# facebookresearch/dmc-net

Measured on AMD Instinct MI355X. Metric: clips/sec (3-seg 224x224) DMC-gen+ResNet-18 train step, higher is better.
Workload: dtype f32

## Files before the change

dmc-net_amd/csrc/conv_x3q.hip:

```cpp
#include "dmc_common.h"
#include "x3s_common.h"
#include <type_traits>
#include <utility>

using namespace dmc;
using namespace dmc::x3;

namespace {

constexpr int QBM = 256, QBN = 64;
constexpr int QWSLOT = 3 * QBN * 32;
constexpr int QWB = 3 * QWSLOT;
constexpr int QEP = 272, QETILE = 32 * QEP;

template <int NW_, int NPB_, int NT_>
struct QG {
    static constexpr int NW = NW_, NPB = NPB_, NT = NT_;
    static constexpr int NA = NW / 2;
    static constexpr int KP = (NT + NA - 1) / NA;
    static constexpr int PT = 3 * KP;
    static constexpr int KW = (18 + NA - 1) / NA;
    static constexpr int ZROW = 32 * NT;
    static constexpr int PSL = (ZROW + 1) * 32;
    static constexpr int PB = 3 * PSL;
// ... 404 lines not shown
int q_choose_tn(long M, int R) {
    const int forced = option(OPT_CONV_CFG);
    if (forced == 201) return 2;
    if (forced == 202) return 1;
    const long n2 = ((M + 255) / 256) * (R / QBN), n1 = ((M + 127) / 128) * (R / QBN);
    const double t2 = (double)((n2 + 255) / 256), t1 = 0.75 * (double)((n1 + 255) / 256);
    return t1 < t2 ? 1 : 2;
}

template <class P, int TN, class GEO>
int launch_q(const X3qArgs& a, hipStream_t s) {
    static LdsLimit lim;
    const hipError_t attr = lim.raise(reinterpret_cast<const void*>(&x3q_conv_kernel<P, TN, GEO>), GEO::LDS);
    if (attr != hipSuccess) return fail(DMC_E_LAUNCH, "x3q_conv: cannot raise the dynamic LDS limit: %s", hipGetErrorString(attr));
    constexpr int BM = 32 * GEO::NW / (2 / TN);
    dim3 grid((a.M + BM - 1) / BM, a.R / QBN);
    x3q_conv_kernel<P, TN, GEO><<<grid, GEO::NW * 64, GEO::LDS, s>>>(a);
    return check_launch("x3q_conv");
}

int q_patch_pixels_max128(long M, int W);
int q_variant(long M, int W, int R) {
    const int forced = option(OPT_CONV_CFG);
    const bool two_ok = q_patch_pixels_max128(M, W) <= QGTwo::ZROW;
    if (forced == 201) return 0;
    if (forced == 202) return 1;
    if (forced == 203 && two_ok) return 2;
    if (forced != 204 && two_ok && ((M + 127) / 128) * (R / QBN) >= 512) return 2;
    return q_choose_tn(M, R) == 2 ? 0 : 1;
}
int q_block_pixels(int variant) { return variant == 0 ? 256 : 128; }


struct X3qWgArgs {
    const void* xq;
    const void* dys;
    float* part;
    int N, OH, Cin, Cout;
    unsigned plane_bytes;
    int steps, per_group, tiles_ci;
};

template <int OW_, int R, int HP_>
struct QWgGeom {
    static constexpr int PW = OW_ + 1;
    static constexpr int D1 = 3, D0 = 2;
    static constexpr int XPL1 = ((D1 * R * PW + 3) / 8) * 8 + 4;
    static constexpr int XPL0 = ((D0 * R * PW + 3) / 8) * 8 + 4;
    static constexpr int NPX = R * OW_;
    static constexpr int NKB = (NPX + 15) / 16;
    static constexpr int DYT = ((NKB * 16 + 31) / 32) * 32;
    static constexpr int DYPL = ((DYT + 3) / 8) * 8 + 4;
    static constexpr int XI = (R * PW + 31) / 32;
    static constexpr int DI = DYT / 32;
    static constexpr int CLS_OFF[4] = {0, 4 * XPL0 * 32, 8 * XPL0 * 32, 8 * XPL0 * 32 + 4 * XPL1 * 32};
    static constexpr int SLB = 8 * XPL0 * 32 + 8 * XPL1 * 32;
    static constexpr int XBYTES = 3 * SLB, DYBYTES = 12 * DYPL * 32;
    static constexpr int LDS = XBYTES + 2 * DYBYTES;
    static_assert(HP_ % R == 0, "steps are whole groups of padded rows");
};

template <int OW_, int R, int HP_>
__global__ __launch_bounds__(768) void x3q_wgrad_kernel(X3qWgArgs a) {
    using G = QWgGeom<OW_, R, HP_>;
    constexpr int PW = G::PW, DYPL = G::DYPL, NKB = G::NKB;
    extern __shared__ __attribute__((aligned(1024))) char lds_qw[];
    const int tid = threadIdx.x, lane = tid & 63;
    const int wave = __builtin_amdgcn_readfirstlane(tid >> 6);
    const int l31 = lane & 31, khalf = lane >> 5, L = lane & 15, grp = (lane >> 4) & 1;
    const int quarter = wave & 3, trow = wave >> 2;
    const int wi = quarter & 1, wj = quarter >> 1;
    const int tci = blockIdx.x % a.tiles_ci, tco = blockIdx.x / a.tiles_ci;
    const unsigned lds0 = lds_addr_of(lds_qw);
    const int s_begin = blockIdx.y * a.per_group;
    const int s_end = s_begin + a.per_group < a.steps ? s_begin + a.per_group : a.steps;
    const u32x4 srd_x = make_srd(a.xq), srd_d = make_srd(a.dys);
    const int nch_in = a.Cin >> 4;
    const int tsl = wave >> 2, tch = wave & 3;
    const unsigned soff_d = (unsigned)(tsl * (a.Cout >> 4) + tco * 4 + tch) * a.plane_bytes;
    const unsigned dplane = lds0 + G::XBYTES + (unsigned)wave * DYPL * 32;
    const int lpx = lane >> 1;
    const unsigned lhalf = (unsigned)(lane & 1) << 4;

    auto pix_off = [&](int g, int x) -> unsigned {
        const int n = g / HP_, y = g - n * HP_ - 1;
        return (g >= 0 && n < a.N && y >= 0 && y < a.OH && x >= 0 && x < OW_) ? (unsigned)((n * a.OH + y) * OW_ + x) * 32u + lhalf : OOB;
    };
    auto issue_x = [&](int q) {
#pragma unroll
        for (int cls = 0; cls < 4; ++cls) {
            const int D = (cls >> 1) ? G::D1 : G::D0, xpl = (cls >> 1) ? G::XPL1 : G::XPL0;
            const int slot0 = (((q % D) + D) % D) * R;
            const unsigned soff_x = (unsigned)(tsl * 4 * nch_in + cls * nch_in + tci * 4 + tch) * a.plane_bytes;
            const unsigned xplane = lds0 + (unsigned)(tsl * G::SLB + G::CLS_OFF[cls] + tch * xpl * 32);
#pragma unroll
            for (int i = 0; i < G::XI; ++i) {
                const int px = 32 * i + lpx;
                const int r = px / PW, col = px - r * PW;
                if (px < R * PW) dma_buf16(srd_x, pix_off(R * q + r, col - 1), soff_x, xplane + (unsigned)(slot0 * PW + 32 * i) * 32u);
            }
        }
    };
    auto issue_dy = [&](int s, int buf) {
#pragma unroll
        for (int i = 0; i < G::DI; ++i) {
            const int p = 32 * i + lpx;
            const int r = p / OW_, x = p - r * OW_;
            dma_buf16(srd_d, p < G::NPX ? pix_off(R * s + r, x) : OOB, soff_d, dplane + (unsigned)buf * G::DYBYTES + (unsigned)(32 * i) * 32u);
        }
    };

    f32x16 acc[3];
#pragma unroll
    for (int t = 0; t < 3; ++t)
#pragma unroll
        for (int e = 0; e < 16; ++e) acc[t][e] = 0.f;

    if (s_begin < s_end) {
        issue_x(s_begin - 1);
        issue_x(s_begin);
        issue_dy(s_begin, 0);
    }
    asm volatile("s_waitcnt vmcnt(0)" ::: "memory");
    __builtin_amdgcn_s_barrier();
    const int py = trow != 1, da = trow == 0 ? -1 : 0;
    const int DR = (py ? G::D1 : G::D0) * R, xpl = py ? G::XPL1 : G::XPL0;
    const int cls_a = py ? G::CLS_OFF[3] : G::CLS_OFF[1];
    const int cls_b = py ? G::CLS_OFF[2] : G::CLS_OFF[0];
    lds_cptr const LB = (lds_cptr)lds_qw;
    int rr[NKB][2], xcol[NKB][2], dyoff[NKB][2];
#pragma unroll
    for (int kb = 0; kb < NKB; ++kb)
#pragma unroll
        for (int u = 0; u < 2; ++u) {
            int P = 16 * kb + 8 * khalf + 4 * u + (L >> 2);
            dyoff[kb][u] = (2 * wi + grp) * DYPL * 32 + G::XBYTES + (L & 3) * 8 + P * 32;
            if (P >= G::NPX) P = G::NPX - 1;
            rr[kb][u] = P / OW_;
            xcol[kb][u] = (2 * wj + grp) * xpl * 32 + (L & 3) * 8 + (P - rr[kb][u] * OW_) * 32;
        }
#pragma unroll 1
    for (int s = s_begin; s < s_end; ++s) {
        const int buf = (s - s_begin) & 1;
        issue_x(s + 1);
        if (s + 1 < s_end) issue_dy(s + 1, buf ^ 1);
        const int sb = (((R * s + da) % DR) + DR) % DR;
#pragma unroll
        for (int kb = 0; kb < NKB; ++kb) {
            int dyo[2], xa[2], xb[2];
#pragma unroll
            for (int u = 0; u < 2; ++u) {
                dyo[u] = dyoff[kb][u] + buf * G::DYBYTES;
                int slot = sb + rr[kb][u];
                slot = slot >= DR ? slot - DR : slot;
                const int xo = xcol[kb][u] + slot * PW * 32;
                xa[u] = xo + cls_a;
                xb[u] = xo + cls_b;
            }
            u32x4 A[3], B[3][3];
#pragma unroll
            for (int sl = 0; sl < 3; ++sl) {
                tr_read2(LB + dyo[0] + sl * 4 * DYPL * 32, LB + dyo[1] + sl * 4 * DYPL * 32, A[sl]);
                tr_read2(LB + xa[0] + sl * G::SLB, LB + xa[1] + sl * G::SLB, B[0][sl]);
                tr_read2(LB + xb[0] + sl * G::SLB + 32, LB + xb[1] + sl * G::SLB + 32, B[1][sl]);
                tr_read2(LB + xa[0] + sl * G::SLB + 32, LB + xa[1] + sl * G::SLB + 32, B[2][sl]);
            }
#pragma unroll
            for (int t = 0; t < 3; ++t) {
                acc[t] = mfma_bf16(A[0], B[t][2], acc[t]);
                acc[t] = mfma_bf16(A[2], B[t][0], acc[t]);
                acc[t] = mfma_bf16(A[1], B[t][1], acc[t]);
                acc[t] = mfma_bf16(A[0], B[t][1], acc[t]);
                acc[t] = mfma_bf16(A[1], B[t][0], acc[t]);
                acc[t] = mfma_bf16(A[0], B[t][0], acc[t]);
            }
        }
        asm volatile("s_waitcnt vmcnt(0) lgkmcnt(0)" ::: "memory");
        __builtin_amdgcn_s_barrier();
    }
    float* out = a.part + (size_t)blockIdx.y * a.Cout * 9 * a.Cin;
    const int ci = tci * 64 + 32 * wj + l31;
#pragma unroll
    for (int t = 0; t < 3; ++t)
#pragma unroll
        for (int e = 0; e < 16; ++e) {
            const int co = tco * 64 + 32 * wi + 8 * (e >> 2) + 4 * khalf + (e & 3);
            out[((size_t)co * 9 + 3 * trow + t) * a.Cin + ci] = acc[t][e];
        }
}

struct X3qWg1Args {
    const void* xq; const void* dys; float* part;
    int Cin, Cout; long Mq; unsigned plane_bytes; int steps, per_group, tiles_ci;
};
constexpr int W1PX = 64, W1PL = 68;
constexpr int W1TILE = 12 * W1PL * 32, W1LDS = 4 * W1TILE;

__global__ __launch_bounds__(256) void x3q_wgrad1_kernel(X3qWg1Args a) {
    extern __shared__ __attribute__((aligned(1024))) char lds_w1[];
    const int tid = threadIdx.x, lane = tid & 63;
    const int wave = __builtin_amdgcn_readfirstlane(tid >> 6);
    const int l31 = lane & 31, khalf = lane >> 5, L = lane & 15, grp = (lane >> 4) & 1;
    const int wi = wave & 1, wj = wave >> 1;
    const int tci = blockIdx.x % a.tiles_ci, tco = blockIdx.x / a.tiles_ci;
    const unsigned lds0 = lds_addr_of(lds_w1);
    const int s_begin = blockIdx.y * a.per_group;
    const int s_end = s_begin + a.per_group < a.steps ? s_begin + a.per_group : a.steps;
    const u32x4 srd_x = make_srd(a.xq), srd_d = make_srd(a.dys);
    const int nch_in = a.Cin >> 4, nch_out = a.Cout >> 4;
    const int lpx = lane >> 1;
    const unsigned lhalf = (unsigned)(lane & 1) << 4;
    auto issue = [&](int s, int buf) {
#pragma unroll
        for (int k = 0; k < 3; ++k) {
            const int pl = 3 * wave + k, sl = pl >> 2, ch = pl & 3;
#pragma unroll
            for (int i = 0; i < 2; ++i) {
                const long p = (long)s * W1PX + 32 * i + lpx;
                const unsigned voff = p < a.Mq ? (unsigned)p * 32u + lhalf : OOB;
                dma_buf16(srd_x, voff, (unsigned)(sl * 4 * nch_in + tci * 4 + ch) * a.plane_bytes,
                          lds0 + (unsigned)(buf * 2 * W1TILE + pl * W1PL * 32 + 32 * i * 32));
                dma_buf16(srd_d, voff, (unsigned)(sl * nch_out + tco * 4 + ch) * a.plane_bytes,
                          lds0 + (unsigned)(buf * 2 * W1TILE + W1TILE + pl * W1PL * 32 + 32 * i * 32));
            }
        }
    };
    f32x16 acc;
#pragma unroll
    for (int e = 0; e < 16; ++e) acc[e] = 0.f;
    if (s_begin < s_end) issue(s_begin, 0);
    asm volatile("s_waitcnt vmcnt(0)" ::: "memory");
    __builtin_amdgcn_s_barrier();
    lds_cptr const LB = (lds_cptr)lds_w1;
#pragma unroll 1
    for (int s = s_begin; s < s_end; ++s) {
        const int buf = (s - s_begin) & 1;
        if (s + 1 < s_end) issue(s + 1, buf ^ 1);
        const int xb = buf * 2 * W1TILE + (2 * wj + grp) * W1PL * 32 + (L & 3) * 8;
        const int db = buf * 2 * W1TILE + W1TILE + (2 * wi + grp) * W1PL * 32 + (L & 3) * 8;
#pragma unroll
        for (int kb = 0; kb < W1PX / 16; ++kb) {
            u32x4 A[3], B[3];
            const int P0 = 16 * kb + 8 * khalf + (L >> 2), P1 = P0 + 4;
#pragma unroll
            for (int sl = 0; sl < 3; ++sl) {
                tr_read2(LB + db + sl * 4 * W1PL * 32 + P0 * 32, LB + db + sl * 4 * W1PL * 32 + P1 * 32, A[sl]);
                tr_read2(LB + xb + sl * 4 * W1PL * 32 + P0 * 32, LB + xb + sl * 4 * W1PL * 32 + P1 * 32, B[sl]);
            }
            acc = mfma_bf16(A[0], B[2], acc);
            acc = mfma_bf16(A[2], B[0], acc);
            acc = mfma_bf16(A[1], B[1], acc);
            acc = mfma_bf16(A[0], B[1], acc);
            acc = mfma_bf16(A[1], B[0], acc);
            acc = mfma_bf16(A[0], B[0], acc);
        }
        asm volatile("s_waitcnt vmcnt(0) lgkmcnt(0)" ::: "memory");
        __builtin_amdgcn_s_barrier();
    }
    float* out = a.part + (size_t)blockIdx.y * a.Cout * a.Cin;
// ... 186 lines not shown
```

dmc-net_amd/csrc/conv_x3s.hip:

```cpp
#include "dmc_common.h"
#include "x3s_common.h"
#include <type_traits>

using namespace dmc;
using namespace dmc::x3;

namespace {

__global__ __launch_bounds__(256) void x3s_split_kernel(const float* __restrict__ x, unsigned short* __restrict__ xs, long M, int C) {
    const int c8 = C >> 3;
    const long total = M * c8;
    const int nchunk = C >> 4;
    for (long o = (long)blockIdx.x * 256 + threadIdx.x; o < total; o += (long)gridDim.x * 256) {
        const long m = o / c8;
        const int g = (int)(o - m * c8);
        const float4 a = reinterpret_cast<const float4*>(x)[2 * o], b = reinterpret_cast<const float4*>(x)[2 * o + 1];
        const float v[8] = {a.x, a.y, a.z, a.w, b.x, b.y, b.z, b.w};
        x3s_store8(xs, v, (size_t)M, nchunk, (size_t)m, g);
    }
}

__global__ __launch_bounds__(256) void x3s_merge_kernel(const unsigned short* __restrict__ xs, float* __restrict__ x, long M, int C) {
    const long total = M * C;
    const size_t plane = (size_t)M * 16;
// ... 389 lines not shown
bool x3s_shape_ok(int N, int H, int W, int K, int R) {
    if (N <= 0 || H <= 0 || W <= 0 || K % 32 != 0 || R % 64 != 0 || K <= 0 || R <= 0) return false;
    const long M = (long)N * H * W;
    return M * (K > R ? K : R) * 6 < (1L << 31);
}

int x3s_choose(int N, int H, int W, int R) {
    const long M = (long)N * H * W;
    const int forced = option(OPT_CONV_CFG);
    if (forced >= 101 && forced <= 105 && patch_pixels_max(N, H, W, X3CFGS[forced - 101].BM) <= X3CFGS[forced - 101].PPMAX) return forced - 101;
    if (forced != 106 && patch_pixels_max(N, H, W, X3CFGS[4].BM) <= X3CFGS[4].PPMAX && ((M + X3CFGS[4].BM - 1) / X3CFGS[4].BM) * (R / 64) >= 512)
        return 4;
    int fallback = -1;
    for (const X3Cfg& c : X3CFGS) {
        if (c.id > 2 || patch_pixels_max(N, H, W, c.BM) > c.PPMAX) continue;
        const long wgs = ((M + c.BM - 1) / c.BM) * (R / 64);
        if (wgs >= 160) return c.id;
        fallback = c.id;
    }
    return fallback;
}

template <int WM, int TM, int PPMAX>
int launch_x3s(const X3Args& a, hipStream_t s) {
    constexpr int BM = 32 * TM * WM;
    constexpr size_t op_bytes = 2 * 3 * PPMAX * 32 + 2 * 3 * 3 * 64 * 32, ep_bytes = 2 * (size_t)BM * 272 + 8192;
    constexpr size_t lds_bytes = op_bytes > ep_bytes ? op_bytes : ep_bytes;
    dim3 grid((a.M + BM - 1) / BM, a.R / 64);
    if ((a.stat_part || a.bnb_part) && a.part_blocks >= 0 && (unsigned)a.part_blocks != grid.x)
        return fail(DMC_E_INVALID, "x3s_conv: statistics partials have %d rows but this launch writes %u (dmc_x3s_conv_stat_blocks was "
                                   "called under another conv_cfg option?)", a.part_blocks, grid.x);
    if constexpr (WM >= 4) {
        if (!(option(OPT_CONV_ABLATE) & 512)) {
            static LdsLimit lim_attr2;
    const hipError_t attr2 = lim_attr2.raise(reinterpret_cast<const void*>(&x3s_conv_kernel<WM, 1, TM, 2, PPMAX, true>), (int)lds_bytes);
            if (attr2 != hipSuccess) return fail(DMC_E_LAUNCH, "x3s_conv: cannot raise the dynamic LDS limit: %s", hipGetErrorString(attr2));
            x3s_conv_kernel<WM, 1, TM, 2, PPMAX, true><<<grid, WM * 64, lds_bytes, s>>>(a);
            return check_launch("x3s_conv");
        }
    }
    static LdsLimit lim_attr;
    const hipError_t attr = lim_attr.raise(reinterpret_cast<const void*>(&x3s_conv_kernel<WM, 1, TM, 2, PPMAX>), (int)lds_bytes);
    if (attr != hipSuccess) return fail(DMC_E_LAUNCH, "x3s_conv: cannot raise the dynamic LDS limit: %s", hipGetErrorString(attr));
    x3s_conv_kernel<WM, 1, TM, 2, PPMAX><<<grid, WM * 64, lds_bytes, s>>>(a);
    return check_launch("x3s_conv");
}

struct X3Bnb { const float *y, *stats, *gamma, *beta; const unsigned char* mask; int relu; double* part; };

int run_x3s(const void* xs, const void* wp, const float* addend, float* y, double* stat_part, int part_blocks, int N, int H, int W,
            int K, int R, hipStream_t s, const X3Bnb* bnb = nullptr) {
    if (!xs || !wp || !y) return fail(DMC_E_INVALID, "x3s_conv: null pointer");
    if (!x3s_shape_ok(N, H, W, K, R)) return fail(DMC_E_INVALID, "x3s_conv: unsupported shape N=%d H=%d W=%d K=%d R=%d", N, H, W, K, R);
    const int cfg = x3s_choose(N, H, W, R);
    X3Args a;
    a.xs = xs; a.wp = wp; a.y = y; a.addend = addend; a.stat_part = stat_part;
    a.N = N; a.H = H; a.W = W; a.K = K; a.R = R; a.M = N * H * W;
    a.plane_bytes = (unsigned)a.M * 32u;
    a.part_blocks = part_blocks;
    if ((stat_part || bnb) && part_blocks <= 0) return fail(DMC_E_INVALID, "x3s_conv: stat_blocks must be the row count of the partials");
    if (bnb) {
        a.bnb_y = bnb->y; a.bnb_stats = bnb->stats; a.bnb_gamma = bnb->gamma; a.bnb_beta = bnb->beta; a.bnb_mask = bnb->mask;
        a.bnb_relu = bnb->relu; a.bnb_part = bnb->part;
    }
    a.ablate = option(OPT_CONV_ABLATE);
    if (DMC_ABL(a.ablate) & 32) a.stat_part = nullptr;
    switch (cfg) {
        case 0: return launch_x3s<8, 1, 608>(a, s);
        case 1: return launch_x3s<4, 1, 320>(a, s);
        case 2: return launch_x3s<2, 1, 192>(a, s);
        case 3: return launch_x3s<4, 2, 608>(a, s);
        case 4: return launch_x3s<4, 1, 225>(a, s);
        default: return fail(DMC_E_INVALID, "x3s_conv: the patch of a %d x %d image does not fit the LDS", H, W);
    }
}

struct X3WgArgs {
    const void* xs;
    const void* dys;
    float* part;
    int N, H, Cin, Cout;
    unsigned plane_bytes;
    int steps, per_group, tiles_ci;
};

template <int W_, int R>
struct WgGeom {
    static constexpr int PW = W_ + 2;
    static constexpr int NGRP = R >= W_ + 2 ? 2 : 4, LA = NGRP / 2;
    static constexpr int NRING = NGRP * R;
    static constexpr int XPX = NRING * PW;
    static constexpr int XPL = ((XPX + 3) / 8) * 8 + 4;
    static constexpr int NPX = R * W_;
    static constexpr int NKB = (NPX + 15) / 16;
    static constexpr int DYP = NKB * 16;
    static constexpr int DYT = ((DYP + 31) / 32) * 32;
    static constexpr int DYPL = ((DYT + 3) / 8) * 8 + 4;
    static constexpr int XI = (R * PW + 31) / 32;
    static constexpr int DI = DYT / 32;
    static constexpr int XBYTES = 12 * XPL * 32, DYBYTES = 12 * DYPL * 32;
    static constexpr int LDS = XBYTES + 2 * DYBYTES;
};

template <int W_, int R>
__global__ __launch_bounds__(768) void x3s_wgrad_kernel(X3WgArgs a) {
    using G = WgGeom<W_, R>;
    constexpr int PW = G::PW, NRING = G::NRING, XPL = G::XPL, DYPL = G::DYPL, NKB = G::NKB;
    extern __shared__ __attribute__((aligned(1024))) char lds_wg[];
    const int tid = threadIdx.x, lane = tid & 63;
    const int wave = __builtin_amdgcn_readfirstlane(tid >> 6);
    const int l31 = lane & 31, khalf = lane >> 5, L = lane & 15, grp = (lane >> 4) & 1;
    const int quarter = wave & 3, trow = wave >> 2;
    const int wi = quarter & 1, wj = quarter >> 1;
    const int tci = blockIdx.x % a.tiles_ci, tco = blockIdx.x / a.tiles_ci;
    const unsigned lds0 = lds_addr_of(lds_wg);
    const int HP = a.H + 2;
    const int s_begin = blockIdx.y * a.per_group;
    const int s_end = s_begin + a.per_group < a.steps ? s_begin + a.per_group : a.steps;
    const u32x4 srd_x = make_srd(a.xs), srd_d = make_srd(a.dys);
    const unsigned soff_x = (unsigned)((wave >> 2) * (a.Cin >> 4) + tci * 4 + (wave & 3)) * a.plane_bytes;
    const unsigned soff_d = (unsigned)((wave >> 2) * (a.Cout >> 4) + tco * 4 + (wave & 3)) * a.plane_bytes;
    const unsigned xplane = lds0 + (unsigned)wave * XPL * 32, dplane = lds0 + G::XBYTES + (unsigned)wave * DYPL * 32;
    const int lpx = lane >> 1;
    const unsigned lhalf = (unsigned)(lane & 1) << 4;

    auto pix_off = [&](int g, int x) -> unsigned {
        const int n = g / HP, y = g - n * HP - 1;
        return (g >= 0 && n < a.N && y >= 0 && y < a.H && x >= 0 && x < W_) ? (unsigned)((n * a.H + y) * W_ + x) * 32u + lhalf : OOB;
    };
    auto issue_x = [&](int q) {
        const int slot0 = (((q % G::NGRP) + G::NGRP) % G::NGRP) * R;
#pragma unroll
        for (int i = 0; i < G::XI; ++i) {
            const int px = 32 * i + lpx;
            const int r = px / PW, col = px - r * PW;
            if (px < R * PW) dma_buf16(srd_x, pix_off(R * q + r, col - 1), soff_x, xplane + (unsigned)(slot0 * PW + 32 * i) * 32u);
        }
    };
    auto issue_dy = [&](int s, int buf) {
#pragma unroll
        for (int i = 0; i < G::DI; ++i) {
            const int p = 32 * i + lpx;
            const int r = p / W_, x = p - r * W_;
            dma_buf16(srd_d, p < G::NPX ? pix_off(R * s + r, x) : OOB, soff_d, dplane + (unsigned)buf * G::DYBYTES + (unsigned)(32 * i) * 32u);
        }
    };

    f32x16 acc[3];
#pragma unroll
    for (int t = 0; t < 3; ++t)
#pragma unroll
        for (int e = 0; e < 16; ++e) acc[t][e] = 0.f;

    if (s_begin < s_end) {
#pragma unroll
        for (int q = -1; q < G::LA; ++q) issue_x(s_begin + q);
        issue_dy(s_begin, 0);
    }
    asm volatile("s_waitcnt vmcnt(0)" ::: "memory");
    __builtin_amdgcn_s_barrier();
    lds_cptr const LB = (lds_cptr)lds_wg;
    int rr[NKB][2], xcol[NKB][2], dyoff[NKB][2];
#pragma unroll
    for (int kb = 0; kb < NKB; ++kb)
#pragma unroll
        for (int u = 0; u < 2; ++u) {
            int P = 16 * kb + 8 * khalf + 4 * u + (L >> 2);
            dyoff[kb][u] = (2 * wi + grp) * DYPL * 32 + G::XBYTES + (L & 3) * 8 + P * 32;
            if (P >= G::NPX) P = G::NPX - 1;
            rr[kb][u] = P / W_;
            xcol[kb][u] = (2 * wj + grp) * XPL * 32 + (L & 3) * 8 + (P - rr[kb][u] * W_) * 32;
        }
#pragma unroll 1
    for (int s = s_begin; s < s_end; ++s) {
        const int buf = (s - s_begin) & 1;
        issue_x(s + G::LA);
        if (s + 1 < s_end) issue_dy(s + 1, buf ^ 1);
        const int sb = (((R * s + trow - 1) % NRING) + NRING) % NRING;
#pragma unroll
        for (int kb = 0; kb < NKB; ++kb) {
            int dyo[2], xo[2];
#pragma unroll
            for (int u = 0; u < 2; ++u) {
                dyo[u] = dyoff[kb][u] + buf * G::DYBYTES;
                int slot = sb + rr[kb][u];
                slot = slot >= NRING ? slot - NRING : slot;
                xo[u] = xcol[kb][u] + slot * PW * 32;
            }
            u32x4 A[3], B[3][3];
#pragma unroll
            for (int sl = 0; sl < 3; ++sl) {
                tr_read2(LB + dyo[0] + sl * 4 * DYPL * 32, LB + dyo[1] + sl * 4 * DYPL * 32, A[sl]);
#pragma unroll
                for (int t = 0; t < 3; ++t)
                    tr_read2(LB + xo[0] + (sl * 4 * XPL + t) * 32, LB + xo[1] + (sl * 4 * XPL + t) * 32, B[t][sl]);
            }
#pragma unroll
            for (int t = 0; t < 3; ++t) {
                acc[t] = mfma_bf16(A[0], B[t][2], acc[t]);
                acc[t] = mfma_bf16(A[2], B[t][0], acc[t]);
                acc[t] = mfma_bf16(A[1], B[t][1], acc[t]);
                acc[t] = mfma_bf16(A[0], B[t][1], acc[t]);
                acc[t] = mfma_bf16(A[1], B[t][0], acc[t]);
                acc[t] = mfma_bf16(A[0], B[t][0], acc[t]);
            }
        }
        asm volatile("s_waitcnt vmcnt(0) lgkmcnt(0)" ::: "memory");
        __builtin_amdgcn_s_barrier();
    }
    float* out = a.part + (size_t)blockIdx.y * a.Cout * 9 * a.Cin;
    const int ci = tci * 64 + 32 * wj + l31;
#pragma unroll
    for (int t = 0; t < 3; ++t)
#pragma unroll
        for (int e = 0; e < 16; ++e) {
            const int co = tco * 64 + 32 * wi + 8 * (e >> 2) + 4 * khalf + (e & 3);
            out[((size_t)co * 9 + 3 * trow + t) * a.Cin + ci] = acc[t][e];
        }
}

__global__ __launch_bounds__(256) void x3s_wgrad_reduce_kernel(const float* __restrict__ part, float* __restrict__ dw, int ngroup, long numel) {
    __shared__ float4 red[16][17];
    const int o = threadIdx.x & 15, sl = threadIdx.x >> 4;
    for (long i0 = (long)blockIdx.x * 64; i0 < numel; i0 += (long)gridDim.x * 64) {
        const long i = i0 + 4 * o;
        float4 s = make_float4(0.f, 0.f, 0.f, 0.f);
        if (i < numel)
            for (int k = sl; k < ngroup; k += 16) {
                const float4 v = *reinterpret_cast<const float4*>(part + (size_t)k * numel + i);
                s.x += v.x; s.y += v.y; s.z += v.z; s.w += v.w;
            }
        red[sl][o] = s;
        __syncthreads();
        if (sl == 0 && i < numel) {
            float4 t = red[0][o];
#pragma unroll
            for (int k = 1; k < 16; ++k) { const float4 v = red[k][o]; t.x += v.x; t.y += v.y; t.z += v.z; t.w += v.w; }
            *reinterpret_cast<float4*>(dw + i) = t;
        }
        __syncthreads();
    }
}

struct X3WgPlan { int R, steps, tiles, groups, per_group; };
bool x3s_wgrad_plan(int N, int H, int W, int Cin, int Cout, X3WgPlan& p) {
    p.R = W == 56 ? 1 : W == 28 ? 2 : W == 14 ? 4 : W == 7 ? 9 : 0;
    if (!p.R || (H + 2) % p.R != 0 || (W == 7 && H != 7) || Cin % 64 != 0 || Cout % 64 != 0) return false;
    p.steps = N * (H + 2) / p.R;
    p.tiles = (Cout / 64) * (Cin / 64);
    int groups = 256 / p.tiles;
    if (groups < 1) groups = 1;
    if (groups > p.steps) groups = p.steps;
    p.per_group = (p.steps + groups - 1) / groups;
    p.groups = (p.steps + p.per_group - 1) / p.per_group;
    return true;
}

template <int W_, int R>
int launch_x3s_wgrad(const X3WgPlan& p, X3WgArgs a, float* dw, hipStream_t s) {
    using G = WgGeom<W_, R>;
    static_assert(G::LDS <= 160 * 1024, "weight-gradient tiles exceed the LDS");
    static LdsLimit lim_attr;
    const hipError_t attr = lim_attr.raise(reinterpret_cast<const void*>(&x3s_wgrad_kernel<W_, R>), G::LDS);
    if (attr != hipSuccess) return fail(DMC_E_LAUNCH, "x3s_wgrad: cannot raise the dynamic LDS limit: %s", hipGetErrorString(attr));
    x3s_wgrad_kernel<W_, R><<<dim3(p.tiles, p.groups), 768, G::LDS, s>>>(a);
    int rc = check_launch("x3s_wgrad");
    if (rc || p.groups == 1) return rc;
    const long numel = (long)a.Cout * 9 * a.Cin;
    const long blocks = (numel + 63) / 64;
    x3s_wgrad_reduce_kernel<<<(int)(blocks > 4096 ? 4096 : blocks), 256, 0, s>>>(a.part, dw, p.groups, numel);
    return check_launch("x3s_wgrad_reduce");
}

__global__ __launch_bounds__(256) void x3s_bnb_final_kernel(const double* __restrict__ part, int nblk, int C,
                                                            float* __restrict__ dgamma, float* __restrict__ dbeta) {
    __shared__ double red[2][4];
    const int c = blockIdx.x, lane = threadIdx.x & 63, wave = threadIdx.x >> 6;
    double s = 0.0, ss = 0.0;
    for (int b = threadIdx.x; b < nblk; b += 256) {
        const double2 v = *reinterpret_cast<const double2*>(part + ((size_t)b * C + c) * 2);
        s += v.x;
        ss += v.y;
    }
#pragma unroll
    for (int o = 32; o > 0; o >>= 1) { s += __shfl_down(s, o, 64); ss += __shfl_down(ss, o, 64); }
    if (lane == 0) { red[0][wave] = s; red[1][wave] = ss; }
    __syncthreads();
    if (threadIdx.x != 0) return;
    dbeta[c] = (float)(red[0][0] + red[0][1] + red[0][2] + red[0][3]);
    dgamma[c] = (float)(red[1][0] + red[1][1] + red[1][2] + red[1][3]);
}

int stream_blocks(long total) {
    long b = (total + 255) / 256;
    return (int)(b < 1 ? 1 : (b > 8192 ? 8192 : b));
}

}

extern "C" {

size_t dmc_x3s_slices_bytes(long M, int C) { return (size_t)M * (size_t)C * 6; }

int dmc_x3s_split(const float* x, void* xs, long M, int C, dmc_stream_t stream) {
    if (!x || !xs || M <= 0 || C <= 0 || C % 16 != 0) return fail(DMC_E_INVALID, "dmc_x3s_split: bad argument");
    x3s_split_kernel<<<stream_blocks(M * (C / 8)), 256, 0, (hipStream_t)stream>>>(x, static_cast<unsigned short*>(xs), M, C);
    return check_launch("x3s_split");
}

int dmc_x3s_merge(const void* xs, float* x, long M, int C, dmc_stream_t stream) {
    if (!x || !xs || M <= 0 || C <= 0 || C % 16 != 0) return fail(DMC_E_INVALID, "dmc_x3s_merge: bad argument");
    x3s_merge_kernel<<<stream_blocks(M * C), 256, 0, (hipStream_t)stream>>>(static_cast<const unsigned short*>(xs), x, M, C);
    return check_launch("x3s_merge");
}

size_t dmc_x3s_wpack_bytes(int Cin, int Cout) { return (size_t)Cin * (size_t)Cout * 9 * 6; }

int dmc_x3s_pack_weights(const float* w, void* wpack_f, void* wpack_t, int Cin, int Cout, dmc_stream_t stream) {
    if (!w || (!wpack_f && !wpack_t) || Cin % 64 != 0 || Cout % 64 != 0 || Cin <= 0 || Cout <= 0)
        return fail(DMC_E_INVALID, "dmc_x3s_pack_weights: bad argument");
    const long total = (long)Cin * Cout * 9;
    x3s_pack_w_kernel<<<dim3(stream_blocks(total) > 1024 ? 1024 : stream_blocks(total), 2), 256, 0, (hipStream_t)stream>>>(
        w, static_cast<unsigned short*>(wpack_f), static_cast<unsigned short*>(wpack_t), Cout, Cin, 1);
    return check_launch("x3s_pack_w");
}

int dmc_x3s_conv_supported(int N, int H, int W, int Cin, int Cout) {
    return Cin % 64 == 0 && Cout % 64 == 0 && x3s_shape_ok(N, H, W, Cin, Cout) && x3s_shape_ok(N, H, W, Cout, Cin) &&
           x3s_choose(N, H, W, Cout) >= 0 && x3s_choose(N, H, W, Cin) >= 0 ? 1 : 0;
}

int dmc_x3s_conv_stat_blocks(int N, int H, int W, int Cout) {
    const int cfg = x3s_choose(N, H, W, Cout);
    if (cfg < 0) return 0;
    const long M = (long)N * H * W;
    return (int)((M + X3CFGS[cfg].BM - 1) / X3CFGS[cfg].BM);
}

int dmc_x3s_conv_fwd(const void* xs, const void* wpack_f, float* y, double* stat_partials, int stat_blocks, int N, int H, int W,
                     int Cin, int Cout, dmc_stream_t stream) {
    return run_x3s(xs, wpack_f, nullptr, y, stat_partials, stat_blocks, N, H, W, Cin, Cout, (hipStream_t)stream);
}

int dmc_x3s_conv_dgrad(const void* dys, const void* wpack_t, const float* addend, float* dx, int N, int H, int W, int Cin, int Cout,
                       dmc_stream_t stream) {
    return run_x3s(dys, wpack_t, addend, dx, nullptr, -1, N, H, W, Cout, Cin, (hipStream_t)stream);
}

int dmc_x3s_conv_wgrad_supported(int N, int H, int W, int Cin, int Cout) {
    X3WgPlan p;
    return x3s_wgrad_plan(N, H, W, Cin, Cout, p) && x3s_shape_ok(N, H, W, Cin, Cout) && x3s_shape_ok(N, H, W, Cout, Cin) ? 1 : 0;
}

size_t dmc_x3s_conv_wgrad_bytes(int N, int H, int W, int Cin, int Cout) {
    X3WgPlan p;
    if (!x3s_wgrad_plan(N, H, W, Cin, Cout, p) || p.groups <= 1) return 0;
    return (size_t)p.groups * Cout * 9 * Cin * sizeof(float);
}

int dmc_x3s_conv_wgrad(const void* xs, const void* dys, float* dw, float* workspace, int N, int H, int W, int Cin, int Cout,
                       dmc_stream_t stream) {
    X3WgPlan p;
    if (!xs || !dys || !dw) return fail(DMC_E_INVALID, "dmc_x3s_conv_wgrad: null pointer");
    if (!dmc_x3s_conv_wgrad_supported(N, H, W, Cin, Cout) || !x3s_wgrad_plan(N, H, W, Cin, Cout, p))
        return fail(DMC_E_INVALID, "dmc_x3s_conv_wgrad: unsupported shape N=%d H=%d W=%d Cin=%d Cout=%d", N, H, W, Cin, Cout);
    if (p.groups > 1 && !workspace) return fail(DMC_E_INVALID, "dmc_x3s_conv_wgrad: workspace required");
    X3WgArgs a;
    a.xs = xs; a.dys = dys; a.part = p.groups > 1 ? workspace : dw;
    a.N = N; a.H = H; a.Cin = Cin; a.Cout = Cout;
    a.plane_bytes = (unsigned)((long)N * H * W) * 32u;
    a.steps = p.steps; a.per_group = p.per_group; a.tiles_ci = Cin / 64;
    hipStream_t s = (hipStream_t)stream;
    switch (W) {
        case 56: return launch_x3s_wgrad<56, 1>(p, a, dw, s);
        case 28: return launch_x3s_wgrad<28, 2>(p, a, dw, s);
        case 14: return launch_x3s_wgrad<14, 4>(p, a, dw, s);
        default: return launch_x3s_wgrad<7, 9>(p, a, dw, s);
    }
}

int dmc_x3s_conv_dgrad_s2_supported(int N, int OH, int OW, int Cin, int Cout) {
    return Cin % 64 == 0 && Cout % 64 == 0 && x3s_shape_ok(N, OH, OW, Cout, Cin) && (long)N * OH * OW * 4 * Cin * 4 < (1L << 40) &&
           patch_pixels_max(N, OH, OW, 128) <= 320 ? 1 : 0;
}

int dmc_x3s_pack_weights_s2(const float* w, void* wpack_t2, int Cin, int Cout, dmc_stream_t stream) {
    if (!w || !wpack_t2 || Cin % 64 != 0 || Cout % 64 != 0 || Cin <= 0 || Cout <= 0)
        return fail(DMC_E_INVALID, "dmc_x3s_pack_weights_s2: bad argument");
    const long total = (long)Cin * Cout * 9;
    x3s_pack_w_kernel<<<dim3(stream_blocks(total) > 1024 ? 1024 : stream_blocks(total), 2), 256, 0, (hipStream_t)stream>>>(
        w, nullptr, static_cast<unsigned short*>(wpack_t2), Cout, Cin, 0);
    return check_launch("x3s_pack_w_s2");
}

int dmc_x3s_conv_dgrad_s2(const void* dys, const void* wpack_t2, float* dx, int N, int OH, int OW, int Cin, int Cout,
                          dmc_stream_t stream) {
    if (!dys || !wpack_t2 || !dx) return fail(DMC_E_INVALID, "dmc_x3s_conv_dgrad_s2: null pointer");
    if (!dmc_x3s_conv_dgrad_s2_supported(N, OH, OW, Cin, Cout))
        return fail(DMC_E_INVALID, "dmc_x3s_conv_dgrad_s2: unsupported shape N=%d OH=%d OW=%d Cin=%d Cout=%d", N, OH, OW, Cin, Cout);
    X3Args a;
    a.xs = dys; a.wp = wpack_t2; a.y = dx; a.addend = nullptr; a.stat_part = nullptr;
    a.N = N; a.H = OH; a.W = OW; a.K = Cout; a.R = Cin; a.M = N * OH * OW;
    a.plane_bytes = (unsigned)a.M * 32u;
    a.ablate = option(OPT_CONV_ABLATE);
    constexpr size_t lds_bytes = 2 * 3 * 320 * 32 + 2 * 3 * 3 * 64 * 32;
    static LdsLimit lim_attr;
    const hipError_t attr = lim_attr.raise(reinterpret_cast<const void*>(&x3s_conv_kernel<4, 1, 1, 2, 320, true, 4>), (int)lds_bytes);
    if (attr != hipSuccess) return fail(DMC_E_LAUNCH, "x3s_conv_dgrad_s2: cannot raise the dynamic LDS limit: %s", hipGetErrorString(attr));
    dim3 grid((a.M + 127) / 128, Cin / 64);
    x3s_conv_kernel<4, 1, 1, 2, 320, true, 4><<<grid, 256, lds_bytes, (hipStream_t)stream>>>(a);
    return check_launch("x3s_conv_dgrad_s2");
}

int dmc_x3s_conv_dgrad_bnb(const void* dys, const void* wpack_t, const float* addend, float* dx, const float* bn_y,
                           const float* bn_stats, const float* bn_gamma, const float* bn_beta, const unsigned char* bn_relu_mask,
                           int bn_relu, double* partials, int stat_blocks, float* dgamma, float* dbeta, int N, int H, int W, int Cin,
                           int Cout, dmc_stream_t stream) {
    if (!bn_y || !bn_stats || !bn_gamma || !bn_beta || !partials || !dgamma || !dbeta)
        return fail(DMC_E_INVALID, "dmc_x3s_conv_dgrad_bnb: null pointer");
    X3Bnb b = {bn_y, bn_stats, bn_gamma, bn_beta, bn_relu_mask, bn_relu, partials};
    int rc = run_x3s(dys, wpack_t, addend, dx, nullptr, stat_blocks, N, H, W, Cout, Cin, (hipStream_t)stream, &b);
    if (rc) return rc;
    x3s_bnb_final_kernel<<<Cin, 256, 0, (hipStream_t)stream>>>(partials, stat_blocks, Cin, dgamma, dbeta);
    return check_launch("x3s_bnb_final");
}

}
```

Before: 3485.

## Software-pipeline LDS fragment reads against MFMA and precompute DMA offsets in wgrad kernels

Both 3x3 weight-gradient kernels now double-buffer the A/B LDS fragments, loading the next fragment while the current MFMAs run, with sched_barriers enforcing the interleave. Per-lane pixel offsets and validity are computed once before the loop, and a row/group cursor advances incrementally, so each step's DMA issue no longer needs the integer divisions inside pix_off. The ring slot index is also updated incrementally. The x3s kernel gains an optional s_memtime instrumentation path behind an ablate flag, and the double buffering raises VGPR use, which could lower occupancy.

```diff
diff --git a/dmc-net_amd/csrc/conv_x3q.hip b/dmc-net_amd/csrc/conv_x3q.hip
--- a/dmc-net_amd/csrc/conv_x3q.hip
+++ b/dmc-net_amd/csrc/conv_x3q.hip
@@ -510,31 +510,59 @@
     const int lpx = lane >> 1;
     const unsigned lhalf = (unsigned)(lane & 1) << 4;
 
-    auto pix_off = [&](int g, int x) -> unsigned {
-        const int n = g / HP_, y = g - n * HP_ - 1;
-        return (g >= 0 && n < a.N && y >= 0 && y < a.OH && x >= 0 && x < OW_) ? (unsigned)((n * a.OH + y) * OW_ + x) * 32u + lhalf : OOB;
+    int xr[G::XI], dr[G::DI];
+    unsigned xv[G::XI], dv[G::DI];
+#pragma unroll
+    for (int i = 0; i < G::XI; ++i) {
+        const int px = 32 * i + lpx;
+        const int r = px / PW, col = px - r * PW - 1;
+        xr[i] = r;
+        xv[i] = (col >= 0 && col < OW_) ? (unsigned)(r * OW_ + col) * 32u + lhalf : OOB + (unsigned)OW_ * 32u;
+    }
+#pragma unroll
+    for (int i = 0; i < G::DI; ++i) {
+        const int p = 32 * i + lpx;
+        dr[i] = p / OW_;
+        dv[i] = p < G::NPX ? (unsigned)p * 32u + lhalf : OOB + (unsigned)OW_ * 32u;
+    }
+    struct Grp { int row, g0; };
+    auto grp_of = [&](int q) -> Grp { const int g = R * (q < 0 ? 0 : q); const int n = g / HP_; return Grp{n * a.OH, g - n * HP_}; };
+    auto grp_next = [&](Grp& p) { p.g0 += R; if (p.g0 >= HP_) { p.g0 = 0; p.row += a.OH; } };
+    auto grp_terms = [&](int q, const Grp& p, unsigned& base, int& bad0, int& bad1, unsigned& sub) {
+        const bool first = p.g0 == 0, live = q >= 0 && q < a.steps;
+        base = (unsigned)((p.row + p.g0) * OW_) * 32u - (first ? 0u : (unsigned)OW_ * 32u);
+        sub = first ? (unsigned)OW_ * 32u : 0u;
+        bad0 = first ? 0 : -1;
+        bad1 = p.g0 + R - 1 > a.OH ? R - 1 : -1;
+        if (!live) { base = 0; bad0 = bad1 = -2; }
+        base = __builtin_amdgcn_readfirstlane(base);
     };
-    auto issue_x = [&](int q) {
+    auto issue_x = [&](int q, int q3, const Grp& p) {
+        unsigned base, sub;
+        int bad0, bad1;
+        grp_terms(q, p, base, bad0, bad1, sub);
+        unsigned v[G::XI];
+#pragma unroll
+        for (int i = 0; i < G::XI; ++i) v[i] = (bad0 == -2 || xr[i] == bad0 || xr[i] == bad1) ? OOB : xv[i] - sub;
 #pragma unroll
         for (int cls = 0; cls < 4; ++cls) {
-            const int D = (cls >> 1) ? G::D1 : G::D0, xpl = (cls >> 1) ? G::XPL1 : G::XPL0;
-            const int slot0 = (((q % D) + D) % D) * R;
+            const int xpl = (cls >> 1) ? G::XPL1 : G::XPL0;
+            const int slot0 = ((cls >> 1) ? q3 : (q & 1)) * R;
             const unsigned soff_x = (unsigned)(tsl * 4 * nch_in + cls * nch_in + tci * 4 + tch) * a.plane_bytes;
             const unsigned xplane = lds0 + (unsigned)(tsl * G::SLB + G::CLS_OFF[cls] + tch * xpl * 32);
 #pragma unroll
-            for (int i = 0; i < G::XI; ++i) {
-                const int px = 32 * i + lpx;
-                const int r = px / PW, col = px - r * PW;
-                if (px < R * PW) dma_buf16(srd_x, pix_off(R * q + r, col - 1), soff_x, xplane + (unsigned)(slot0 * PW + 32 * i) * 32u);
-            }
+            for (int i = 0; i < G::XI; ++i)
+                if (32 * i + lpx < R * PW) dma_buf16(srd_x, v[i], soff_x + base, xplane + (unsigned)(slot0 * PW + 32 * i) * 32u);
         }
     };
-    auto issue_dy = [&](int s, int buf) {
+    auto issue_dy = [&](int s, const Grp& p, int buf) {
+        unsigned base, sub;
+        int bad0, bad1;
+        grp_terms(s, p, base, bad0, bad1, sub);
 #pragma unroll
         for (int i = 0; i < G::DI; ++i) {
-            const int p = 32 * i + lpx;
-            const int r = p / OW_, x = p - r * OW_;
-            dma_buf16(srd_d, p < G::NPX ? pix_off(R * s + r, x) : OOB, soff_d, dplane + (unsigned)buf * G::DYBYTES + (unsigned)(32 * i) * 32u);
+            const unsigned v = (bad0 == -2 || dr[i] == bad0 || dr[i] == bad1) ? OOB : dv[i] - sub;
+            dma_buf16(srd_d, v, soff_d + base, dplane + (unsigned)buf * G::DYBYTES + (unsigned)(32 * i) * 32u);
         }
     };
 
@@ -544,10 +572,17 @@
 #pragma unroll
         for (int e = 0; e < 16; ++e) acc[t][e] = 0.f;
 
+    Grp gx = grp_of(s_begin - 1), gd = grp_of(s_begin);
+    int q3 = (s_begin + 2) % 3;
     if (s_begin < s_end) {
-        issue_x(s_begin - 1);
-        issue_x(s_begin);
-        issue_dy(s_begin, 0);
+        issue_x(s_begin - 1, q3, gx);
+        if (s_begin > 0) grp_next(gx);
+        q3 = q3 == 2 ? 0 : q3 + 1;
+        issue_x(s_begin, q3, gx);
+        grp_next(gx);
+        q3 = q3 == 2 ? 0 : q3 + 1;
+        issue_dy(s_begin, gd, 0);
+        grp_next(gd);
     }
     asm volatile("s_waitcnt vmcnt(0)" ::: "memory");
     __builtin_amdgcn_s_barrier();
@@ -565,44 +600,70 @@
             dyoff[kb][u] = (2 * wi + grp) * DYPL * 32 + G::XBYTES + (L & 3) * 8 + P * 32;
             if (P >= G::NPX) P = G::NPX - 1;
             rr[kb][u] = P / OW_;
-            xcol[kb][u] = (2 * wj + grp) * xpl * 32 + (L & 3) * 8 + (P - rr[kb][u] * OW_) * 32;
-        }
+            xcol[kb][u] = (2 * wj + grp) * xpl * 32 + (L & 3) * 8 + (P - rr[kb][u] * OW_) * 32 + rr[kb][u] * PW * 32;
+        }
+    int sb = (((R * s_begin + da) % DR) + DR) % DR;
 #pragma unroll 1
     for (int s = s_begin; s < s_end; ++s) {
         const int buf = (s - s_begin) & 1;
-        issue_x(s + 1);
-        if (s + 1 < s_end) issue_dy(s + 1, buf ^ 1);
-        const int sb = (((R * s + da) % DR) + DR) % DR;
-#pragma unroll
-        for (int kb = 0; kb < NKB; ++kb) {
-            int dyo[2], xa[2], xb[2];
+        u32x4 A[2][3], B[2][3];
+        int dyo[2], xa[2], xb[2];
+        auto frag_addr = [&](int kb) {
 #pragma unroll
             for (int u = 0; u < 2; ++u) {
                 dyo[u] = dyoff[kb][u] + buf * G::DYBYTES;
-                int slot = sb + rr[kb][u];
-                slot = slot >= DR ? slot - DR : slot;
-                const int xo = xcol[kb][u] + slot * PW * 32;
+                const int xo = xcol[kb][u] + (rr[kb][u] >= DR - sb ? (sb - DR) * PW * 32 : sb * PW * 32);
                 xa[u] = xo + cls_a;
                 xb[u] = xo + cls_b;
             }
-            u32x4 A[3], B[3][3];
+        };
+        auto read_a = [&](u32x4 (&Af)[3]) {
+#pragma unroll
+            for (int sl = 0; sl < 3; ++sl) tr_read2(LB + dyo[0] + sl * 4 * DYPL * 32, LB + dyo[1] + sl * 4 * DYPL * 32, Af[sl]);
+        };
+        auto read_b = [&](int t, u32x4 (&Bf)[3]) {
 #pragma unroll
             for (int sl = 0; sl < 3; ++sl) {
-                tr_read2(LB + dyo[0] + sl * 4 * DYPL * 32, LB + dyo[1] + sl * 4 * DYPL * 32, A[sl]);
-                tr_read2(LB + xa[0] + sl * G::SLB, LB + xa[1] + sl * G::SLB, B[0][sl]);
-                tr_read2(LB + xb[0] + sl * G::SLB + 32, LB + xb[1] + sl * G::SLB + 32, B[1][sl]);
-                tr_read2(LB + xa[0] + sl * G::SLB + 32, LB + xa[1] + sl * G::SLB + 32, B[2][sl]);
-            }
+                if (t == 0) tr_read2(LB + xa[0] + sl * G::SLB, LB + xa[1] + sl * G::SLB, Bf[sl]);
+                else if (t == 1) tr_read2(LB + xb[0] + sl * G::SLB + 32, LB + xb[1] + sl * G::SLB + 32, Bf[sl]);
+                else tr_read2(LB + xa[0] + sl * G::SLB + 32, LB + xa[1] + sl * G::SLB + 32, Bf[sl]);
+            }
+        };
+        frag_addr(0);
+        read_a(A[0]);
+        read_b(0, B[0]);
+        __builtin_amdgcn_sched_barrier(0);
+        issue_x(s + 1, q3, gx);
+        grp_next(gx);
+        q3 = q3 == 2 ? 0 : q3 + 1;
+        if (s + 1 < s_end) issue_dy(s + 1, gd, buf ^ 1);
+        grp_next(gd);
+        __builtin_amdgcn_sched_barrier(0);
+#pragma unroll
+        for (int kb = 0; kb < NKB; ++kb)
 #pragma unroll
             for (int t = 0; t < 3; ++t) {
-                acc[t] = mfma_bf16(A[0], B[t][2], acc[t]);
-                acc[t] = mfma_bf16(A[2], B[t][0], acc[t]);
-                acc[t] = mfma_bf16(A[1], B[t][1], acc[t]);
-                acc[t] = mfma_bf16(A[0], B[t][1], acc[t]);
-                acc[t] = mfma_bf16(A[1], B[t][0], acc[t]);
-                acc[t] = mfma_bf16(A[0], B[t][0], acc[t]);
-            }
-        }
+                const int st = 3 * kb + t;
+                if (t < 2) {
+                    read_b(t + 1, B[(st + 1) & 1]);
+                } else if (kb + 1 < NKB) {
+                    frag_addr(kb + 1);
+                    read_a(A[(kb + 1) & 1]);
+                    read_b(0, B[(st + 1) & 1]);
+                }
+                __builtin_amdgcn_sched_barrier(0);
+                const u32x4(&Af)[3] = A[kb & 1];
+                const u32x4(&Bf)[3] = B[st & 1];
+                acc[t] = mfma_bf16(Af[0], Bf[2], acc[t]);
+                acc[t] = mfma_bf16(Af[2], Bf[0], acc[t]);
+                acc[t] = mfma_bf16(Af[1], Bf[1], acc[t]);
+                acc[t] = mfma_bf16(Af[0], Bf[1], acc[t]);
+                acc[t] = mfma_bf16(Af[1], Bf[0], acc[t]);
+                acc[t] = mfma_bf16(Af[0], Bf[0], acc[t]);
+                __builtin_amdgcn_sched_barrier(0);
+            }
+        sb += R;
+        sb = sb >= DR ? sb - DR : sb;
         asm volatile("s_waitcnt vmcnt(0) lgkmcnt(0)" ::: "memory");
         __builtin_amdgcn_s_barrier();
     }
diff --git a/dmc-net_amd/csrc/conv_x3s.hip b/dmc-net_amd/csrc/conv_x3s.hip
--- a/dmc-net_amd/csrc/conv_x3s.hip
+++ b/dmc-net_amd/csrc/conv_x3s.hip
@@ -495,6 +495,7 @@
     int N, H, Cin, Cout;
     unsigned plane_bytes;
     int steps, per_group, tiles_ci;
+    int ablate;
 };
 
 template <int W_, int R>
@@ -537,25 +538,52 @@
     const int lpx = lane >> 1;
     const unsigned lhalf = (unsigned)(lane & 1) << 4;
 
-    auto pix_off = [&](int g, int x) -> unsigned {
-        const int n = g / HP, y = g - n * HP - 1;
-        return (g >= 0 && n < a.N && y >= 0 && y < a.H && x >= 0 && x < W_) ? (unsigned)((n * a.H + y) * W_ + x) * 32u + lhalf : OOB;
-    };
-    auto issue_x = [&](int q) {
-        const int slot0 = (((q % G::NGRP) + G::NGRP) % G::NGRP) * R;
+    int xr[G::XI], dr[G::DI];
+    unsigned xv[G::XI], dv[G::DI];
+#pragma unroll
+    for (int i = 0; i < G::XI; ++i) {
+        const int px = 32 * i + lpx;
+        const int r = px / PW, col = px - r * PW - 1;
+        xr[i] = r;
+        xv[i] = (col >= 0 && col < W_) ? (unsigned)(r * W_ + col) * 32u + lhalf : OOB + (unsigned)W_ * 32u;
+    }
+#pragma unroll
+    for (int i = 0; i < G::DI; ++i) {
+        const int p = 32 * i + lpx;
+        dr[i] = p / W_;
+        dv[i] = p < G::NPX ? (unsigned)p * 32u + lhalf : OOB + (unsigned)W_ * 32u;
+    }
+    struct Grp { int row, g0; };
+    auto grp_of = [&](int q) -> Grp { const int g = R * (q < 0 ? 0 : q); const int n = g / HP; return Grp{n * a.H, g - n * HP}; };
+    auto grp_next = [&](Grp& p) { p.g0 += R; if (p.g0 >= HP) { p.g0 = 0; p.row += a.H; } };
+    auto grp_terms = [&](int q, const Grp& p, unsigned& base, int& bad0, int& bad1, unsigned& sub) {
+        const bool first = p.g0 == 0, live = q >= 0 && q < a.steps;
+        base = (unsigned)((p.row + p.g0) * W_) * 32u - (first ? 0u : (unsigned)W_ * 32u);
+        sub = first ? (unsigned)W_ * 32u : 0u;
+        bad0 = first ? 0 : -1;
+        bad1 = p.g0 + R == HP ? R - 1 : -1;
+        if (!live) { base = 0; bad0 = bad1 = -2; }
+        base = __builtin_amdgcn_readfirstlane(base);
+    };
+    auto issue_x = [&](int q, const Grp& p) {
+        const int slot0 = (q & (G::NGRP - 1)) * R;
+        unsigned base, sub;
+        int bad0, bad1;
+        grp_terms(q, p, base, bad0, bad1, sub);
 #pragma unroll
         for (int i = 0; i < G::XI; ++i) {
-            const int px = 32 * i + lpx;
-            const int r = px / PW, col = px - r * PW;
-            if (px < R * PW) dma_buf16(srd_x, pix_off(R * q + r, col - 1), soff_x, xplane + (unsigned)(slot0 * PW + 32 * i) * 32u);
-        }
-    };
-    auto issue_dy = [&](int s, int buf) {
+            const unsigned v = (bad0 == -2 || xr[i] == bad0 || xr[i] == bad1) ? OOB : xv[i] - sub;
+            if (32 * i + lpx < R * PW) dma_buf16(srd_x, v, soff_x + base, xplane + (unsigned)(slot0 * PW + 32 * i) * 32u);
+        }
+    };
+    auto issue_dy = [&](int s, const Grp& p, int buf) {
+        unsigned base, sub;
+        int bad0, bad1;
+        grp_terms(s, p, base, bad0, bad1, sub);
 #pragma unroll
         for (int i = 0; i < G::DI; ++i) {
-            const int p = 32 * i + lpx;
-            const int r = p / W_, x = p - r * W_;
-            dma_buf16(srd_d, p < G::NPX ? pix_off(R * s + r, x) : OOB, soff_d, dplane + (unsigned)buf * G::DYBYTES + (unsigned)(32 * i) * 32u);
+            const unsigned v = (bad0 == -2 || dr[i] == bad0 || dr[i] == bad1) ? OOB : dv[i] - sub;
+            dma_buf16(srd_d, v, soff_d + base, dplane + (unsigned)buf * G::DYBYTES + (unsigned)(32 * i) * 32u);
         }
     };
 
@@ -565,10 +593,15 @@
 #pragma unroll
         for (int e = 0; e < 16; ++e) acc[t][e] = 0.f;
 
+    Grp gx = grp_of(s_begin - 1), gd = grp_of(s_begin);
     if (s_begin < s_end) {
 #pragma unroll
-        for (int q = -1; q < G::LA; ++q) issue_x(s_begin + q);
-        issue_dy(s_begin, 0);
+        for (int q = -1; q < G::LA; ++q) {
+            issue_x(s_begin + q, gx);
+            if (s_begin + q >= 0) grp_next(gx);
+        }
+        issue_dy(s_begin, gd, 0);
+        grp_next(gd);
     }
     asm volatile("s_waitcnt vmcnt(0)" ::: "memory");
     __builtin_amdgcn_s_barrier();
@@ -582,46 +615,79 @@
             dyoff[kb][u] = (2 * wi + grp) * DYPL * 32 + G::XBYTES + (L & 3) * 8 + P * 32;
             if (P >= G::NPX) P = G::NPX - 1;
             rr[kb][u] = P / W_;
-            xcol[kb][u] = (2 * wj + grp) * XPL * 32 + (L & 3) * 8 + (P - rr[kb][u] * W_) * 32;
-        }
+            xcol[kb][u] = (2 * wj + grp) * XPL * 32 + (L & 3) * 8 + (P - rr[kb][u] * W_) * 32 + rr[kb][u] * PW * 32;
+        }
+    int sb = (((R * s_begin + trow - 1) % NRING) + NRING) % NRING;
+    [[maybe_unused]] long long tim[3] = {0, 0, 0}, t0 = 0, t1 = 0, t2 = 0;
 #pragma unroll 1
     for (int s = s_begin; s < s_end; ++s) {
         const int buf = (s - s_begin) & 1;
-        issue_x(s + G::LA);
-        if (s + 1 < s_end) issue_dy(s + 1, buf ^ 1);
-        const int sb = (((R * s + trow - 1) % NRING) + NRING) % NRING;
-#pragma unroll
-        for (int kb = 0; kb < NKB; ++kb) {
-            int dyo[2], xo[2];
+        if (DMC_ABL(a.ablate & 2048)) t0 = (long long)__builtin_amdgcn_s_memtime();
+        u32x4 A[2][3], B[2][3];
+        int dyo[2], xo[2];
+        auto frag_addr = [&](int kb) {
 #pragma unroll
             for (int u = 0; u < 2; ++u) {
                 dyo[u] = dyoff[kb][u] + buf * G::DYBYTES;
-                int slot = sb + rr[kb][u];
-                slot = slot >= NRING ? slot - NRING : slot;
-                xo[u] = xcol[kb][u] + slot * PW * 32;
+                xo[u] = xcol[kb][u] + (rr[kb][u] >= NRING - sb ? (sb - NRING) * PW * 32 : sb * PW * 32);
             }
-            u32x4 A[3], B[3][3];
-#pragma unroll
-            for (int sl = 0; sl < 3; ++sl) {
-                tr_read2(LB + dyo[0] + sl * 4 * DYPL * 32, LB + dyo[1] + sl * 4 * DYPL * 32, A[sl]);
-#pragma unroll
-                for (int t = 0; t < 3; ++t)
-                    tr_read2(LB + xo[0] + (sl * 4 * XPL + t) * 32, LB + xo[1] + (sl * 4 * XPL + t) * 32, B[t][sl]);
+        };
+        auto read_a = [&](u32x4 (&Af)[3]) {
+#pragma unroll
+            for (int sl = 0; sl < 3; ++sl) tr_read2(LB + dyo[0] + sl * 4 * DYPL * 32, LB + dyo[1] + sl * 4 * DYPL * 32, Af[sl]);
+        };
+        auto read_b = [&](int t, u32x4 (&Bf)[3]) {
+#pragma unroll
+            for (int sl = 0; sl < 3; ++sl) tr_read2(LB + xo[0] + (sl * 4 * XPL + t) * 32, LB + xo[1] + (sl * 4 * XPL + t) * 32, Bf[sl]);
+        };
+        frag_addr(0);
+        read_a(A[0]);
+        read_b(0, B[0]);
+        __builtin_amdgcn_sched_barrier(0);
+        issue_x(s + G::LA, gx);
+        grp_next(gx);
+        if (s + 1 < s_end) issue_dy(s + 1, gd, buf ^ 1);
+        grp_next(gd);
+        __builtin_amdgcn_sched_barrier(0);
+        if (DMC_ABL(a.ablate & 2048)) { t1 = (long long)__builtin_amdgcn_s_memtime(); __builtin_amdgcn_sched_barrier(0); }
+#pragma unroll
+        for (int kb = 0; kb < NKB; ++kb)
+#pragma unroll
+            for (int t = 0; t < 3; ++t) {
+                const int st = 3 * kb + t;
+                if (t < 2) {
+                    read_b(t + 1, B[(st + 1) & 1]);
+                } else if (kb + 1 < NKB) {
+                    frag_addr(kb + 1);
+                    read_a(A[(kb + 1) & 1]);
+                    read_b(0, B[(st + 1) & 1]);
+                }
+                __builtin_amdgcn_sched_barrier(0);
+                const u32x4(&Af)[3] = A[kb & 1];
+                const u32x4(&Bf)[3] = B[st & 1];
+                acc[t] = mfma_bf16(Af[0], Bf[2], acc[t]);
+                acc[t] = mfma_bf16(Af[2], Bf[0], acc[t]);
+                acc[t] = mfma_bf16(Af[1], Bf[1], acc[t]);
+                acc[t] = mfma_bf16(Af[0], Bf[1], acc[t]);
+                acc[t] = mfma_bf16(Af[1], Bf[0], acc[t]);
+                acc[t] = mfma_bf16(Af[0], Bf[0], acc[t]);
+                __builtin_amdgcn_sched_barrier(0);
             }
-#pragma unroll
-            for (int t = 0; t < 3; ++t) {
-                acc[t] = mfma_bf16(A[0], B[t][2], acc[t]);
-                acc[t] = mfma_bf16(A[2], B[t][0], acc[t]);
-                acc[t] = mfma_bf16(A[1], B[t][1], acc[t]);
-                acc[t] = mfma_bf16(A[0], B[t][1], acc[t]);
-                acc[t] = mfma_bf16(A[1], B[t][0], acc[t]);
-                acc[t] = mfma_bf16(A[0], B[t][0], acc[t]);
-            }
-        }
+        sb += R;
+        sb = sb >= NRING ? sb - NRING : sb;
+        if (DMC_ABL(a.ablate & 2048)) t2 = (long long)__builtin_amdgcn_s_memtime();
         asm volatile("s_waitcnt vmcnt(0) lgkmcnt(0)" ::: "memory");
         __builtin_amdgcn_s_barrier();
+        if (DMC_ABL(a.ablate & 2048)) {
+            const long long t3 = (long long)__builtin_amdgcn_s_memtime();
+            tim[0] += t1 - t0; tim[1] += t2 - t1; tim[2] += t3 - t2;
+        }
     }
     float* out = a.part + (size_t)blockIdx.y * a.Cout * 9 * a.Cin;
+    if (DMC_ABL(a.ablate & 2048) && blockIdx.x == 0) {
+        if (lane < 4) out[4 * wave + lane] = lane < 3 ? (float)tim[lane] : (float)(s_end - s_begin);
+        return;
+    }
     const int ci = tci * 64 + 32 * wj + l31;
 #pragma unroll
     for (int t = 0; t < 3; ++t)
@@ -783,6 +849,7 @@
     a.N = N; a.H = H; a.Cin = Cin; a.Cout = Cout;
     a.plane_bytes = (unsigned)((long)N * H * W) * 32u;
     a.steps = p.steps; a.per_group = p.per_group; a.tiles_ci = Cin / 64;
+    a.ablate = option(OPT_CONV_ABLATE);
     hipStream_t s = (hipStream_t)stream;
     switch (W) {
         case 56: return launch_x3s_wgrad<56, 1>(p, a, dw, s);
```

Result: no change. 3501 (median of 6 runs) (+0.4%).
